# alex-petrenko/sample-factory

Measured on AMD Instinct MI355X. Metric: env-steps/sec (whole node), 4096 envs, 84x84x4 obs, higher is better.
Workload: dtype f32

## Files before the change

### sample_factory_amd/csrc/sf_nn_wimg.h

```cpp
#pragma once

template <int CIN, int HH, int WW, int KS, int ST, int KSPLIT>
struct WimgGeom {
    static constexpr int OH = (HH - KS) / ST + 1, OW = (WW - KS) / ST + 1, P = OH * OW, STEPS = (P + 3) / 4, TAPS = KS * KS;
    static constexpr int CT = CIN / 16, TAPS_W = TAPS / KSPLIT, NW = 4 * KSPLIT;
    static constexpr int XB = HH * WW * CIN * 4, YB = P * 64 * 4;
    static constexpr int XI = (XB + 1023) / 1024, YI = (4 * STEPS * 256 + 1023) / 1024;
    static constexpr int XSLOT = XI * 1024, YSLOT = YI * 1024, STAGE = XSLOT + YSLOT;
    static constexpr int NI = (XI + YI + NW - 1) / NW;
    static constexpr int PMAX = 4 * STEPS - 1;
    static constexpr int XREACH = (((ST * (PMAX / OW) + KS - 1) * WW + ST * (PMAX % OW) + KS - 1) * CIN + CIN) * 4;
    static_assert(CT == 2 || CT == 4, "Cin = 32 or 64: one float2 / float4 per lane");
    static_assert(TAPS % KSPLIT == 0 && TAPS_W % KS == 0, "a wave's tap group is whole filter rows");
    static_assert(XREACH <= STAGE, "padded-pixel reads must stay inside the stage");
    static_assert(2 * STAGE <= 160 * 1024 / (KSPLIT == 1 ? 2 : 1), "LDS: two work-groups per CU (4 waves) or one (8 waves)");
};

template <int CIN, int HH, int WW, int KS, int ST, int KSPLIT>
__global__ __launch_bounds__(256 * KSPLIT, 2) void k_wgrad_img(const float *__restrict__ in, int64_t in_stride,
                                                               const float *__restrict__ dy, float *__restrict__ partial,
                                                               float *__restrict__ partial_b, int nsamples) {
    typedef WimgGeom<CIN, HH, WW, KS, ST, KSPLIT> G;
    constexpr int OW = G::OW, STEPS = G::STEPS, TAPS_W = G::TAPS_W, CT = G::CT, NW = G::NW, N = 64, K = G::TAPS * CIN;
    constexpr int XB = G::XB, YB = G::YB, XI = G::XI, NI = G::NI, XSLOT = G::XSLOT, STAGE = G::STAGE;
    typedef float fvec __attribute__((ext_vector_type(CT)));
    __shared__ __attribute__((aligned(1024))) char lds[2 * STAGE];
    const int tid = threadIdx.x, lane = tid & 63, wave = __builtin_amdgcn_readfirstlane(tid >> 6);
    const int i16 = lane & 15, kg = lane >> 4;
    const int nt = wave & 3, ks = wave >> 2;
    const int per = (nsamples + (int)gridDim.x - 1) / (int)gridDim.x;
    const int s_beg = (int)blockIdx.x * per, s_end = min(nsamples, s_beg + per);
    f32x4 acc[TAPS_W][CT];
#pragma unroll
    for (int t = 0; t < TAPS_W; ++t)
#pragma unroll
        for (int j = 0; j < CT; ++j) acc[t][j] = f32x4{0.f, 0.f, 0.f, 0.f};
    float bsum = 0.f;
    if (s_beg < s_end) {
        int doff[NI];
        bool is_y[NI];
#pragma unroll
        for (int j = 0; j < NI; ++j) {
            const int q = wave + NW * j;
            is_y[j] = q >= XI;
            const int b = (is_y[j] ? q - XI : q) * 1024 + lane * 16;
            doff[j] = (b < (is_y[j] ? YB : XB)) ? b : -1;
        }
        const char *inb = reinterpret_cast<const char *>(in), *dyb = reinterpret_cast<const char *>(dy);
        const char *zero = reinterpret_cast<const char *>(sf_zero_page) + (lane & 7) * 16;
        auto issue = [&](int s, int stage) {
            const char *xs = inb + (int64_t)s * in_stride * 4, *ys = dyb + (int64_t)s * YB;
            char *st = lds + stage * STAGE;
#pragma unroll
            for (int j = 0; j < NI; ++j) {
                const int q = wave + NW * j;
                if (q < XI + G::YI) {
                    const char *src = doff[j] < 0 ? zero : (is_y[j] ? ys : xs) + doff[j];
                    GLDS16(src, st + (is_y[j] ? XSLOT + (q - XI) * 1024 : q * 1024));
                }
            }
        };
        const int tapbase = ks * (TAPS_W / KS) * WW * CIN * 4;
        int xo[STEPS];
#pragma unroll
        for (int st = 0; st < STEPS; ++st) {
            const int p = 4 * st + kg, oh = p / OW, ow = p - oh * OW;
            xo[st] = ((ST * oh * WW + ST * ow) * CIN + CT * i16) * 4 + tapbase;
        }
        const int yo = XSLOT + kg * 256 + (16 * nt + i16) * 4;

        auto sample = [&](auto stage_c) {
            constexpr int SOFF = decltype(stage_c)::value * STAGE;
#pragma unroll
            for (int st = 0; st < STEPS; ++st) {
                const float b = *reinterpret_cast<const float *>(lds + SOFF + yo + st * 1024);
                bsum += b;
#pragma unroll
                for (int t = 0; t < TAPS_W; ++t) {
                    const int imm = SOFF + ((t / KS) * WW + (t % KS)) * CIN * 4;
                    const fvec a = *reinterpret_cast<const fvec *>(__builtin_assume_aligned(lds + xo[st] + imm, 4 * CT));
#pragma unroll
                    for (int j = 0; j < CT; ++j)
                        acc[t][j] = __builtin_amdgcn_mfma_f32_16x16x4f32(a[j], b, acc[t][j], 0, 0, 0);
                }
            }
        };
        issue(s_beg, 0);
        for (int s = s_beg; s < s_end; s += 2) {
            asm volatile("s_waitcnt vmcnt(0)" ::: "memory");
            __syncthreads();
            if (s + 1 < s_end) issue(s + 1, 1);
            sample(std::integral_constant<int, 0>{});
            if (s + 1 < s_end) {
                asm volatile("s_waitcnt vmcnt(0)" ::: "memory");
                __syncthreads();
                if (s + 2 < s_end) issue(s + 2, 0);
                sample(std::integral_constant<int, 1>{});
            }
        }
    }
    float *dst = partial + (int64_t)blockIdx.x * K * N + 16 * nt + i16;
#pragma unroll
    for (int t = 0; t < TAPS_W; ++t)
#pragma unroll
        for (int j = 0; j < CT; ++j)
#pragma unroll
            for (int r = 0; r < 4; ++r) dst[((ks * TAPS_W + t) * CIN + CT * (4 * kg + r) + j) * N] = acc[t][j][r];
    if (partial_b && ks == 0) {
        bsum += __shfl_xor(bsum, 16, 64);
        bsum += __shfl_xor(bsum, 32, 64);
        if (kg == 0) partial_b[(int64_t)blockIdx.x * N + 16 * nt + i16] = bsum;
    }
}
```

Before: 2.091 million.

## Stagger k-split waves in wgrad kernel and interleave DMA issue with MFMAs

Measured after the change: 2.114 million, median of 6. 1.1% higher.

```diff
diff --git a/sample_factory_amd/csrc/sf_nn_wimg.h b/sample_factory_amd/csrc/sf_nn_wimg.h
--- a/sample_factory_amd/csrc/sf_nn_wimg.h
+++ b/sample_factory_amd/csrc/sf_nn_wimg.h
@@ -14,7 +14,32 @@
     static_assert(TAPS % KSPLIT == 0 && TAPS_W % KS == 0, "a wave's tap group is whole filter rows");
     static_assert(XREACH <= STAGE, "padded-pixel reads must stay inside the stage");
     static_assert(2 * STAGE <= 160 * 1024 / (KSPLIT == 1 ? 2 : 1), "LDS: two work-groups per CU (4 waves) or one (8 waves)");
+    static constexpr bool piece_is_whole(int j) {
+        for (int w = 0; w < NW; ++w) {
+            const int q = w + NW * j;
+            if (q < XI ? (q + 1) * 1024 > XB : (q - XI + 1) * 1024 > YB) return false;
+        }
+        return true;
+    }
+    static constexpr bool pieces_whole_but_last() {
+        for (int j = 0; j + 1 < NI; ++j)
+            if (!piece_is_whole(j)) return false;
+        return true;
+    }
 };
+
+__device__ __forceinline__ void wimg_glds16_on(const void *ubase, uint32_t voff, uint32_t lds_byte_addr, uint32_t on) {
+    uint64_t keep;
+    asm volatile("s_mov_b64 %0, exec\n\ts_cmp_lg_u32 %4, 0\n\ts_cselect_b64 exec, exec, 0\n\ts_mov_b32 m0, %3\n\ts_nop 0\n\t"
+                 "global_load_lds_dwordx4 %1, %2\n\ts_mov_b64 exec, %0"
+                 : "=&s"(keep) : "v"(voff), "s"(ubase), "s"(lds_byte_addr), "s"(on) : "memory", "m0", "scc");
+}
+__device__ __forceinline__ void wimg_glds16_on(const void *src, uint32_t lds_byte_addr, uint32_t on) {
+    uint64_t keep;
+    asm volatile("s_mov_b64 %0, exec\n\ts_cmp_lg_u32 %3, 0\n\ts_cselect_b64 exec, exec, 0\n\ts_mov_b32 m0, %2\n\ts_nop 0\n\t"
+                 "global_load_lds_dwordx4 %1, off\n\ts_mov_b64 exec, %0"
+                 : "=&s"(keep) : "v"(src), "s"(lds_byte_addr), "s"(on) : "memory", "m0", "scc");
+}
 
 template <int CIN, int HH, int WW, int KS, int ST, int KSPLIT>
 __global__ __launch_bounds__(256 * KSPLIT, 2) void k_wgrad_img(const float *__restrict__ in, int64_t in_stride,
@@ -69,33 +94,125 @@
         }
         const int yo = XSLOT + kg * 256 + (16 * nt + i16) * 4;
 
-        auto sample = [&](auto stage_c) {
-            constexpr int SOFF = decltype(stage_c)::value * STAGE;
-#pragma unroll
-            for (int st = 0; st < STEPS; ++st) {
-                const float b = *reinterpret_cast<const float *>(lds + SOFF + yo + st * 1024);
-                bsum += b;
-#pragma unroll
-                for (int t = 0; t < TAPS_W; ++t) {
-                    const int imm = SOFF + ((t / KS) * WW + (t % KS)) * CIN * 4;
-                    const fvec a = *reinterpret_cast<const fvec *>(__builtin_assume_aligned(lds + xo[st] + imm, 4 * CT));
-#pragma unroll
-                    for (int j = 0; j < CT; ++j)
-                        acc[t][j] = __builtin_amdgcn_mfma_f32_16x16x4f32(a[j], b, acc[t][j], 0, 0, 0);
-                }
-            }
-        };
-        issue(s_beg, 0);
-        for (int s = s_beg; s < s_end; s += 2) {
-            asm volatile("s_waitcnt vmcnt(0)" ::: "memory");
-            __syncthreads();
-            if (s + 1 < s_end) issue(s + 1, 1);
-            sample(std::integral_constant<int, 0>{});
-            if (s + 1 < s_end) {
+        if constexpr (KSPLIT == 2) {
+            constexpr int H0 = (STEPS + 1) / 2, ROWS = TAPS_W / KS;
+            static_assert(XB % 1024 == 0 && NW * (NI - 1) >= XI && G::pieces_whole_but_last(),
+                          "only a wave's last piece, a dY piece, has zero-page lanes");
+            const int cnt = s_end - s_beg;
+            const uint32_t lds0 = (uint32_t)(uintptr_t)(__attribute__((address_space(3))) char *)lds;
+            int xb[2][ROWS][STEPS], yb[2];
+#pragma unroll
+            for (int g = 0; g < 2; ++g) {
+                yb[g] = g * STAGE + yo;
+                asm("" : "+v"(yb[g]));
+#pragma unroll
+                for (int r = 0; r < ROWS; ++r)
+#pragma unroll
+                    for (int st = 0; st < STEPS; ++st) {
+                        xb[g][r][st] = g * STAGE + xo[st] + r * WW * CIN * 4;
+                        asm("" : "+v"(xb[g][r][st]));
+                    }
+            }
+            const char *zy = doff[NI - 1] < 0 ? zero : dyb + doff[NI - 1];
+            const uint32_t zs = doff[NI - 1] < 0 ? 0u : (uint32_t)YB;
+            auto half = [&](auto hc, auto gc, int i) {
+                constexpr int HF = decltype(hc)::value, STG = decltype(gc)::value, Q0 = HF ? H0 : 0, Q1 = HF ? STEPS : H0;
+                static_assert(2 * (Q1 - Q0) >= NI, "two DMA pieces per quad cover a wave's share of the next sample");
+                const uint32_t load = __builtin_amdgcn_readfirstlane(ks != HF && i + 1 < cnt ? 1 : 0);
+                const uint32_t load_last = __builtin_amdgcn_readfirstlane(load && wave + NW * (NI - 1) < XI + G::YI ? 1 : 0);
+                const uint32_t sn = (uint32_t)(s_beg + i + 1);
+                const char *xs = inb + (int64_t)sn * in_stride * 4, *ys = dyb + (int64_t)sn * YB;
+                const uint32_t dst = lds0 + (1 - STG) * STAGE;
+                fvec a[2][TAPS_W];
+                float b[2];
+                auto fetch = [&](int st, int slot) {
+                    b[slot] = *reinterpret_cast<const float *>(lds + yb[STG] + st * 1024);
+#pragma unroll
+                    for (int t = 0; t < TAPS_W; ++t)
+                        a[slot][t] = *reinterpret_cast<const fvec *>(
+                            __builtin_assume_aligned(lds + xb[STG][t / KS][st] + (t % KS) * CIN * 4, 4 * CT));
+                };
+                auto mfmas = [&](int slot, int t0, int t1) {
+#pragma unroll
+                    for (int t = t0; t < t1; ++t)
+#pragma unroll
+                        for (int j = 0; j < CT; ++j) {
+                            acc[t][j] = __builtin_amdgcn_mfma_f32_16x16x4f32(a[slot][t][j], b[slot], acc[t][j], 0, 0, 0);
+                            asm volatile("" : "+v"(acc[t][j]));
+                        }
+                };
+                fetch(Q0, 0);
+#pragma unroll
+                for (int st = Q0; st < Q1; ++st) {
+                    const int slot = (st - Q0) & 1;
+                    bsum += b[slot];
+                    mfmas(slot, 0, TAPS_W / 2);
+                    __builtin_amdgcn_sched_barrier(0);
+                    if (st + 1 < Q1) fetch(st + 1, slot ^ 1);
+#pragma unroll
+                    for (int j = 2 * (st - Q0); j < 2 * (st - Q0) + 2 && j < NI; ++j) {
+                        const int q = wave + NW * j;
+                        const uint32_t to = dst + (is_y[j] ? XSLOT + (q - XI) * 1024 : q * 1024);
+                        if (G::piece_is_whole(j)) wimg_glds16_on(is_y[j] ? ys : xs, (uint32_t)doff[j], to, load);
+                        else {
+                            wimg_glds16_on(zy + (uint64_t)sn * zs, to, load_last);
+                        }
+                    }
+                    __builtin_amdgcn_sched_barrier(0);
+                    mfmas(slot, TAPS_W / 2, TAPS_W);
+                    __builtin_amdgcn_sched_barrier(0);
+                }
+            };
+            auto phase_barrier = [&]() {
                 asm volatile("s_waitcnt vmcnt(0)" ::: "memory");
                 __syncthreads();
-                if (s + 2 < s_end) issue(s + 2, 0);
-                sample(std::integral_constant<int, 1>{});
+            };
+            std::integral_constant<int, 0> c0;
+            std::integral_constant<int, 1> c1;
+            issue(s_beg, 0);
+            if (ks == 1) phase_barrier();
+            for (int i = 0; i < cnt; i += 2) {
+                phase_barrier();
+                half(c0, c0, i);
+                phase_barrier();
+                half(c1, c0, i);
+                if (i + 1 < cnt) {
+                    phase_barrier();
+                    half(c0, c1, i + 1);
+                    phase_barrier();
+                    half(c1, c1, i + 1);
+                }
+            }
+            if (ks == 0) phase_barrier();
+        } else {
+            auto sample = [&](auto stage_c) {
+                constexpr int SOFF = decltype(stage_c)::value * STAGE;
+#pragma unroll
+                for (int st = 0; st < STEPS; ++st) {
+                    const float b = *reinterpret_cast<const float *>(lds + SOFF + yo + st * 1024);
+                    bsum += b;
+#pragma unroll
+                    for (int t = 0; t < TAPS_W; ++t) {
+                        const int imm = SOFF + ((t / KS) * WW + (t % KS)) * CIN * 4;
+                        const fvec a = *reinterpret_cast<const fvec *>(__builtin_assume_aligned(lds + xo[st] + imm, 4 * CT));
+#pragma unroll
+                        for (int j = 0; j < CT; ++j)
+                            acc[t][j] = __builtin_amdgcn_mfma_f32_16x16x4f32(a[j], b, acc[t][j], 0, 0, 0);
+                    }
+                }
+            };
+            issue(s_beg, 0);
+            for (int s = s_beg; s < s_end; s += 2) {
+                asm volatile("s_waitcnt vmcnt(0)" ::: "memory");
+                __syncthreads();
+                if (s + 1 < s_end) issue(s + 1, 1);
+                sample(std::integral_constant<int, 0>{});
+                if (s + 1 < s_end) {
+                    asm volatile("s_waitcnt vmcnt(0)" ::: "memory");
+                    __syncthreads();
+                    if (s + 2 < s_end) issue(s + 2, 0);
+                    sample(std::integral_constant<int, 1>{});
+                }
             }
         }
     }
```
